# reedrosenbluth/LASS

Measured on AMD Instinct MI355X. Metric: clips/sec (10s@16kHz), higher is better.
Workload: dtype f32; 1 GPU; ResUNet30 separate() fp32, batch=16/GPU, 10s@16kHz clips, fixed precomputed condition embedding, seeded random-init weights (BASELINE configs[1]); samples_per_clip=160000, parallelism=clip-sharded x1

## Files before the change

lass_amd/csrc/pw_gemm_split_body.h:

```cpp
    __shared__ __attribute__((aligned(16))) bf16x8 lds[2][2][3][SPLANE];
    const int tid = threadIdx.x, lane = tid & 63, wave = tid >> 6;
    const int wn = wave >> 1, wp = wave & 1;
    int bx, by, b;
    block_coords(p, bx, by, b);
    const int n0 = by * NB;
    const unsigned P = (unsigned)p.H * (unsigned)p.W;
    const unsigned p0 = (unsigned)bx * PB;
    const int K = TCONV ? p.Cin : p.Cin2;
    const unsigned Nw = (unsigned)p.Nw;

    const int sc = tid & (NB - 1), so = __builtin_amdgcn_readfirstlane(tid >> 7);
    const float* xs = (TCONV ? p.in + (size_t)b * p.in_bs : p.in2 + (size_t)b * p.in2_bs) + min(p0 + (unsigned)sc, P - 1u) +
                      (size_t)(so * 8) * P;
    const size_t wplane = (size_t)(K / 8) * Nw;
    const bf16x8* ws = reinterpret_cast<const bf16x8*>(sw.w) + (XI ? (size_t)b * 3 * wplane : (size_t)0) + (size_t)so * Nw + n0 + sc;
    const float* psc = TCONV ? p.pro_scale + so * 8 : nullptr;
    const float* psh = TCONV ? p.pro_shift + (size_t)b * p.pro_shift_bs + so * 8 : nullptr;
    struct Act {
        float s[8], h[8];
    };
    struct Stage {
        float x[8];
        bf16x8 w[3];
        Act a;
    };
    Stage S0, S1;
    Act T;
    const auto aload = [&](Act& a, int ch) {
        if (TCONV) {
#pragma unroll
            for (int j = 0; j < 8; ++j) {
                a.s[j] = psc[(size_t)ch * KC + j];
                a.h[j] = psh[(size_t)ch * KC + j];
            }
        }
    };
    const auto gload = [&](Stage& st, int ch) {
        const size_t k = (size_t)ch * KC;
#pragma unroll
        for (int j = 0; j < 8; ++j) st.x[j] = xs[(k + j) * P];
#pragma unroll
        for (int pc = 0; pc < 3; ++pc) st.w[pc] = ws[pc * wplane + (size_t)ch * (KC / 8) * Nw];
    };
    const auto sstore = [&](const Stage& st, int buf) {
        float x[8];
#pragma unroll
        for (int j = 0; j < 8; ++j) x[j] = TCONV ? leaky(fmaf(st.x[j], st.a.s[j], st.a.h[j])) : st.x[j];
        bf16x8 xp[3];
        split3(x, xp[0], xp[1], xp[2]);
#pragma unroll
        for (int pc = 0; pc < 3; ++pc) {
            lds[buf][0][pc][so * NB + sc] = st.w[pc];
            lds[buf][1][pc][so * PB + sc] = xp[pc];
        }
    };

    f32x16 acc[2][2];
    if constexpr (XI)
        acc_zero(acc);
    else
        acc_init<TCONV>(p, acc, n0, wn, lane);
    f32x16 accs[2][2];
    if constexpr (ACC2) acc_zero(accs);

    const int fo = (lane >> 5) * NB + (lane & 31);
    const auto mma = [&](int buf) {
        bf16x8 fa[3][2], fb[3][2];
#pragma unroll
        for (int pc = 0; pc < 3; ++pc)
#pragma unroll
            for (int t = 0; t < 2; ++t) {
                fa[pc][t] = lds[buf][0][pc][fo + wn * 64 + t * 32];
                fb[pc][t] = lds[buf][1][pc][fo + wp * 64 + t * 32];
            }
        __builtin_amdgcn_sched_barrier(0);
        constexpr int WP[6] = {2, 0, 1, 1, 0, 0}, XP[6] = {0, 2, 1, 0, 1, 0};
#pragma unroll
        for (int t = 0; t < 6; ++t) {
            if constexpr (ACC2) {
                if (t < 5) {
                    accs[0][0] = __builtin_amdgcn_mfma_f32_32x32x16_bf16(fa[WP[t]][0], fb[XP[t]][0], accs[0][0], 0, 0, 0);
                    accs[0][1] = __builtin_amdgcn_mfma_f32_32x32x16_bf16(fa[WP[t]][0], fb[XP[t]][1], accs[0][1], 0, 0, 0);
                    accs[1][0] = __builtin_amdgcn_mfma_f32_32x32x16_bf16(fa[WP[t]][1], fb[XP[t]][0], accs[1][0], 0, 0, 0);
                    accs[1][1] = __builtin_amdgcn_mfma_f32_32x32x16_bf16(fa[WP[t]][1], fb[XP[t]][1], accs[1][1], 0, 0, 0);
                    continue;
                }
            }
            acc[0][0] = __builtin_amdgcn_mfma_f32_32x32x16_bf16(fa[WP[t]][0], fb[XP[t]][0], acc[0][0], 0, 0, 0);
            acc[0][1] = __builtin_amdgcn_mfma_f32_32x32x16_bf16(fa[WP[t]][0], fb[XP[t]][1], acc[0][1], 0, 0, 0);
            acc[1][0] = __builtin_amdgcn_mfma_f32_32x32x16_bf16(fa[WP[t]][1], fb[XP[t]][0], acc[1][0], 0, 0, 0);
            acc[1][1] = __builtin_amdgcn_mfma_f32_32x32x16_bf16(fa[WP[t]][1], fb[XP[t]][1], acc[1][1], 0, 0, 0);
        }
        __builtin_amdgcn_sched_barrier(0);
    };
    const int nch = K / KC;
    aload(S0.a, 0);
    aload(S1.a, 1);
    gload(S0, 0);
    gload(S1, 1);
    sstore(S0, 0);
    aload(S0.a, min(2, nch - 1));
    gload(S0, min(2, nch - 1));
    __syncthreads();
    for (int ch = 0; ch < nch; ch += 2) {
        aload(T, min(ch + 3, nch - 1));
        mma(0);
        sstore(S1, 1);
        S1.a = T;
        gload(S1, min(ch + 3, nch - 1));
        __syncthreads();
        aload(T, min(ch + 4, nch - 1));
        mma(1);
        sstore(S0, 0);
        S0.a = T;
        gload(S0, min(ch + 4, nch - 1));
        __syncthreads();
    }
    if constexpr (ACC2) {
#pragma unroll
        for (int i = 0; i < 2; ++i)
#pragma unroll
            for (int j = 0; j < 2; ++j)
#pragma unroll
                for (int r = 0; r < 16; ++r) acc[i][j][r] += accs[i][j][r];
    }
    store_tile<TCONV>(p, acc, b, n0, p0, P, wn, wp, lane);
```

Baseline: 1171 clips/s.

## Interleave LDS stores, global loads and VALU prep with MFMA via sched_group_barrier

```diff
diff --git a/lass_amd/csrc/pw_gemm_split_body.h b/lass_amd/csrc/pw_gemm_split_body.h
--- a/lass_amd/csrc/pw_gemm_split_body.h
+++ b/lass_amd/csrc/pw_gemm_split_body.h
@@ -25,7 +25,6 @@
         Act a;
     };
     Stage S0, S1;
-    Act T;
     const auto aload = [&](Act& a, int ch) {
         if (TCONV) {
 #pragma unroll
@@ -42,12 +41,13 @@
 #pragma unroll
         for (int pc = 0; pc < 3; ++pc) st.w[pc] = ws[pc * wplane + (size_t)ch * (KC / 8) * Nw];
     };
-    const auto sstore = [&](const Stage& st, int buf) {
+    const auto sprep = [&](const Stage& st, bf16x8 (&xp)[3]) {
         float x[8];
 #pragma unroll
         for (int j = 0; j < 8; ++j) x[j] = TCONV ? leaky(fmaf(st.x[j], st.a.s[j], st.a.h[j])) : st.x[j];
-        bf16x8 xp[3];
         split3(x, xp[0], xp[1], xp[2]);
+    };
+    const auto swrite = [&](const Stage& st, const bf16x8 (&xp)[3], int buf) {
 #pragma unroll
         for (int pc = 0; pc < 3; ++pc) {
             lds[buf][0][pc][so * NB + sc] = st.w[pc];
@@ -64,32 +64,49 @@
     if constexpr (ACC2) acc_zero(accs);
 
     const int fo = (lane >> 5) * NB + (lane & 31);
-    const auto mma = [&](int buf) {
+    constexpr int WP[6] = {2, 0, 1, 1, 0, 0}, XP[6] = {0, 2, 1, 0, 1, 0};
+    const auto prod = [&](const bf16x8 (&fa)[3][2], const bf16x8 (&fb)[3][2], int t) {
+        f32x16(&d)[2][2] = (ACC2 && t < 5) ? accs : acc;
+        d[0][0] = __builtin_amdgcn_mfma_f32_32x32x16_bf16(fa[WP[t]][0], fb[XP[t]][0], d[0][0], 0, 0, 0);
+        d[0][1] = __builtin_amdgcn_mfma_f32_32x32x16_bf16(fa[WP[t]][0], fb[XP[t]][1], d[0][1], 0, 0, 0);
+        d[1][0] = __builtin_amdgcn_mfma_f32_32x32x16_bf16(fa[WP[t]][1], fb[XP[t]][0], d[1][0], 0, 0, 0);
+        d[1][1] = __builtin_amdgcn_mfma_f32_32x32x16_bf16(fa[WP[t]][1], fb[XP[t]][1], d[1][1], 0, 0, 0);
+    };
+    constexpr int NV = TCONV ? 9 : 7;
+    const auto phase = [&](int buf, Stage& st, int chn) {
         bf16x8 fa[3][2], fb[3][2];
+        bf16x8 xp[3];
+        constexpr int RW[3] = {2, 0, 1}, RX[3] = {0, 2, 1};
 #pragma unroll
-        for (int pc = 0; pc < 3; ++pc)
+        for (int g = 0; g < 3; ++g) {
 #pragma unroll
-            for (int t = 0; t < 2; ++t) {
-                fa[pc][t] = lds[buf][0][pc][fo + wn * 64 + t * 32];
-                fb[pc][t] = lds[buf][1][pc][fo + wp * 64 + t * 32];
-            }
+            for (int t = 0; t < 2; ++t) fa[RW[g]][t] = lds[buf][0][RW[g]][fo + wn * 64 + t * 32];
+#pragma unroll
+            for (int t = 0; t < 2; ++t) fb[RX[g]][t] = lds[buf][1][RX[g]][fo + wp * 64 + t * 32];
+            __builtin_amdgcn_sched_barrier(0);
+        }
+        prod(fa, fb, 0);
+        prod(fa, fb, 1);
+        prod(fa, fb, 2);
+        sprep(st, xp);
+#pragma unroll
+        for (int i = 0; i < 12; ++i) {
+            __builtin_amdgcn_sched_group_barrier(0x008, 1, 0);
+            __builtin_amdgcn_sched_group_barrier(0x002, NV, 0);
+        }
         __builtin_amdgcn_sched_barrier(0);
-        constexpr int WP[6] = {2, 0, 1, 1, 0, 0}, XP[6] = {0, 2, 1, 0, 1, 0};
+        aload(st.a, chn);
+        __builtin_amdgcn_sched_barrier(0);
+        prod(fa, fb, 3);
+        prod(fa, fb, 4);
+        prod(fa, fb, 5);
+        swrite(st, xp, buf ^ 1);
+        gload(st, chn);
 #pragma unroll
-        for (int t = 0; t < 6; ++t) {
-            if constexpr (ACC2) {
-                if (t < 5) {
-                    accs[0][0] = __builtin_amdgcn_mfma_f32_32x32x16_bf16(fa[WP[t]][0], fb[XP[t]][0], accs[0][0], 0, 0, 0);
-                    accs[0][1] = __builtin_amdgcn_mfma_f32_32x32x16_bf16(fa[WP[t]][0], fb[XP[t]][1], accs[0][1], 0, 0, 0);
-                    accs[1][0] = __builtin_amdgcn_mfma_f32_32x32x16_bf16(fa[WP[t]][1], fb[XP[t]][0], accs[1][0], 0, 0, 0);
-                    accs[1][1] = __builtin_amdgcn_mfma_f32_32x32x16_bf16(fa[WP[t]][1], fb[XP[t]][1], accs[1][1], 0, 0, 0);
-                    continue;
-                }
-            }
-            acc[0][0] = __builtin_amdgcn_mfma_f32_32x32x16_bf16(fa[WP[t]][0], fb[XP[t]][0], acc[0][0], 0, 0, 0);
-            acc[0][1] = __builtin_amdgcn_mfma_f32_32x32x16_bf16(fa[WP[t]][0], fb[XP[t]][1], acc[0][1], 0, 0, 0);
-            acc[1][0] = __builtin_amdgcn_mfma_f32_32x32x16_bf16(fa[WP[t]][1], fb[XP[t]][0], acc[1][0], 0, 0, 0);
-            acc[1][1] = __builtin_amdgcn_mfma_f32_32x32x16_bf16(fa[WP[t]][1], fb[XP[t]][1], acc[1][1], 0, 0, 0);
+        for (int i = 0; i < 12; ++i) {
+            __builtin_amdgcn_sched_group_barrier(0x008, 1, 1);
+            if (i < 6) __builtin_amdgcn_sched_group_barrier(0x200, 1, 1);
+            if (i >= 1) __builtin_amdgcn_sched_group_barrier(0x020, 1, 1);
         }
         __builtin_amdgcn_sched_barrier(0);
     };
@@ -98,24 +115,22 @@
     aload(S1.a, 1);
     gload(S0, 0);
     gload(S1, 1);
-    sstore(S0, 0);
+    {
+        bf16x8 xp[3];
+        sprep(S0, xp);
+        swrite(S0, xp, 0);
+    }
     aload(S0.a, min(2, nch - 1));
     gload(S0, min(2, nch - 1));
     __syncthreads();
-    for (int ch = 0; ch < nch; ch += 2) {
-        aload(T, min(ch + 3, nch - 1));
-        mma(0);
-        sstore(S1, 1);
-        S1.a = T;
-        gload(S1, min(ch + 3, nch - 1));
+    int ch = 0;
+    do {
+        phase(0, S1, min(ch + 3, nch - 1));
         __syncthreads();
-        aload(T, min(ch + 4, nch - 1));
-        mma(1);
-        sstore(S0, 0);
-        S0.a = T;
-        gload(S0, min(ch + 4, nch - 1));
+        phase(1, S0, min(ch + 4, nch - 1));
         __syncthreads();
-    }
+        ch += 2;
+    } while (ch < nch);
     if constexpr (ACC2) {
 #pragma unroll
         for (int i = 0; i < 2; ++i)
```

Measured after the change: 1185 clips/s, median of 6. 1.01x the previous value.
